# aikiriao/AAD

Measured on AMD Instinct MI355X. Metric: Msamples/s encode+decode, 48 kHz stereo 4-bit, higher is better.
Workload: dtype int32

## Files before the change

aad_amd/capi.py:

```python
import ctypes as C
import os

import numpy as np


class AADApiResult:
    OK = 0
    INVALID_ARGUMENT = 1
    INVALID_FORMAT = 2
    INSUFFICIENT_BUFFER = 3
    INSUFFICIENT_DATA = 4
    PARAMETER_NOT_SET = 5
    NG = 6
    _names = {0: "OK", 1: "INVALID_ARGUMENT", 2: "INVALID_FORMAT", 3: "INSUFFICIENT_BUFFER",
              4: "INSUFFICIENT_DATA", 5: "PARAMETER_NOT_SET", 6: "NG"}

    @classmethod
    def name(cls, v):
        return cls._names.get(int(v), str(v))


class AADHeaderInfo(C.Structure):
    _fields_ = [("format_version", C.c_uint32), ("codec_version", C.c_uint32),
                ("num_channels", C.c_uint16), ("num_samples", C.c_uint32),
# ... 23 lines not shown

class AADHipPlanarOutput(C.Structure):
    _fields_ = [("sample_type", C.c_int32), ("reserved", C.c_uint32), ("stream_stride", C.c_uint64), ("channel_stride", C.c_uint64)]


class AADHipRowStats(C.Structure):
    _fields_ = [("sum_sq", C.c_uint64), ("sum_abs", C.c_uint64), ("max_abs", C.c_uint64), ("count", C.c_uint64)]


class AADHipLaneState(C.Structure):
    _fields_ = [("weight", C.c_int32 * 4), ("history", C.c_int32 * 4),
                ("stepsize_index", C.c_int32), ("quantize_error", C.c_int32)]


STREAM_DESC_DTYPE = np.dtype([("pcm_offset", "<u8"), ("data_offset", "<u8"), ("data_size", "<u8"),
                              ("num_samples", "<u4"), ("reserved", "<u4")])
ERROR_STATS_DTYPE = np.dtype([("rms_error", "<f8"), ("mean_abs_error", "<f8"), ("max_abs_error", "<f8")])
WINDOW_DTYPE = np.dtype([("stream", "<i8"), ("first_frame", "<i8")])
SAMPLE_INT16, SAMPLE_FLOAT32 = 0, 1
RECONSTRUCT_DECODED, RECONSTRUCT_RESIDUAL = 0, 1
OPTION_LANE_MAPPING, OPTION_TRIAL_LANES, OPTION_STAGING_THREADS, OPTION_TILE_KBYTES, OPTION_COMPARE_ORDER = 0, 1, 2, 3, 4
LANE_MAPPINGS = {"auto": 0, "dense": 1, "quad": 2, "quad-fused": 3, "dense-tiled": 4}
TRIAL_LANES = {"dual": 0, "single": 1}
LANE_STATE_DTYPE = np.dtype([("weight", "<i4", (4,)), ("history", "<i4", (4,)),
                             ("stepsize_index", "<i4"), ("quantize_error", "<i4")])

_PKG_DIR = os.path.dirname(os.path.abspath(__file__))
LIBRARY_PATH = os.environ.get("AAD_HIP_LIBRARY", os.path.join(_PKG_DIR, "libaad_hip.so"))

LEGACY_SYMBOLS = [
    "AADEncoder_CalculateBlockSize", "AADEncoder_EncodeHeader", "AADEncoder_CalculateWorkSize",
    "AADEncoder_Create", "AADEncoder_Destroy", "AADEncoder_SetEncodeParameter", "AADEncoder_EncodeWhole",
    "AADDecoder_DecodeHeader", "AADDecoder_CalculateWorkSize", "AADDecoder_Create", "AADDecoder_Destroy",
    "AADDecoder_SetHeader", "AADDecoder_DecodeBlock", "AADDecoder_DecodeWhole",
]
HIP_SYMBOLS = [
    "AADHip_GetDeviceCount", "AADHip_ContextCreate", "AADHip_ContextDestroy", "AADHip_ContextSynchronize",
    "AADHip_ContextLastError", "AADHip_ContextSignalNextRun", "AADHip_SignalNextRunSupported", "AADHip_ContextSetOption", "AADHip_CalculateEncodedSize", "AADHip_EncodePlanCreate",
    "AADHip_EncodePlanDestroy", "AADHip_EncodePlanRun", "AADHip_DecodePlanCreate", "AADHip_DecodePlanDestroy",
    "AADHip_DecodePlanRun", "AADHip_EncodeBatch", "AADHip_DecodeBatch",
    "AADHip_ReconstructPlanCreate", "AADHip_ReconstructPlanDestroy", "AADHip_ReconstructPlanRun",
    "AADHip_ReconstructBatch", "AADHip_SegmentedEncodePlanCreate", "AADHip_SegmentedEncodeBatch",
    "AADHip_SegmentedReconstructPlanCreate", "AADHip_SegmentedReconstructBatch",
    "AADHip_WindowDecodePlanCreate", "AADHip_WindowDecodePlanDestroy", "AADHip_WindowDecodePlanRun",
    "AADHip_WindowDecodePlanRunStats", "AADHip_MixedWindowDecodePlanCreate", "AADHip_ChannelMixWindowDecodePlanCreate",
    "AADHip_PlanarEncodePlanCreate", "AADHip_PlanarEncodePlanRun",
# ... 257 lines not shown
```

aad_amd/csrc/aad_decode_split.hip:

```cpp
#include <cstring>

#include "aad_decode_split.hip.h"
#include "aad_launch.h"

namespace aad {

template <int BITS, bool LDSRES>
static void launch_bits(const SplitDecodeArgs &sa, dim3 grid, dim3 block, hipStream_t stream)
{
  if (sa.d.channels == 1)
    AAD_LAUNCH((decode_split_kernel<BITS, 1, false, LDSRES>), grid, block, 0, stream, sa);
  else if (sa.d.mid_side)
    AAD_LAUNCH((decode_split_kernel<BITS, 2, true, LDSRES>), grid, block, 0, stream, sa);
  else
    AAD_LAUNCH((decode_split_kernel<BITS, 2, false, LDSRES>), grid, block, 0, stream, sa);
}

void launch_decode_split(const DecodeArgs &args, const DecodeLaunch &p, int32_t *residual, hipStream_t stream)
{
  SplitDecodeArgs sa;
  sa.d = args;
  sa.residual = residual;
  sa.residual_stride = p.residual_stride;
  sa.reserved = 0;
  const dim3 grid(p.grid), block(p.workgroup);
  const bool lds = p.kernel == DecodeKernel::SplitLds;
  switch (args.bits) {
    case 4: lds ? launch_bits<4, true>(sa, grid, block, stream) : launch_bits<4, false>(sa, grid, block, stream); break;
    case 3: lds ? launch_bits<3, true>(sa, grid, block, stream) : launch_bits<3, false>(sa, grid, block, stream); break;
    default: lds ? launch_bits<2, true>(sa, grid, block, stream) : launch_bits<2, false>(sa, grid, block, stream); break;
  }
}

}

#if AAD_PHASE_TIMING
extern "C" uint32_t AADHipDebug_ReadSplitPhaseTimes(uint64_t *out, uint32_t capacity)
{
  uint32_t n = 0, zero = 0;
  uint64_t host[512];
  (void)hipDeviceSynchronize();
  (void)hipMemcpyFromSymbol(&n, HIP_SYMBOL(aad::g_phase_count), sizeof(n));
  (void)hipMemcpyFromSymbol(host, HIP_SYMBOL(aad::g_phase_times), sizeof(host));
  (void)hipMemcpyToSymbol(HIP_SYMBOL(aad::g_phase_count), &zero, sizeof(zero));
  if (n > capacity) n = capacity;
  memcpy(out, host, sizeof(uint64_t) * n);
  return n;
}
#endif
```

aad_amd/csrc/aad_decode_split.hip.h:

```cpp
#ifndef AAD_DECODE_SPLIT_HIP_H
#define AAD_DECODE_SPLIT_HIP_H

#include "aad_decode.hip.h"

namespace aad {

struct SplitDecodeArgs {
  DecodeArgs d;
  int32_t *residual;
  uint32_t residual_stride;
  uint32_t reserved;
};

struct BlockRef {
  const uint8_t *src;
  uint64_t pcm_first;
  uint32_t n;
  uint32_t avail;
};

__device__ __forceinline__ BlockRef locate_block(const DecodeArgs &a, uint64_t g, uint32_t ch)
{
  uint32_t s;
  StreamDesc sd;
  uint64_t b;
  if (a.uni.enabled) {
    s = (uint32_t)g / a.uni.blocks_per_stream;
    b = (uint32_t)g - s * a.uni.blocks_per_stream;
    sd = uniform_stream(a.uni, s);
  } else {
    s = find_stream(a.block_prefix, a.num_streams, g);
    sd = a.streams[s];
    b = g - a.block_prefix[s];
  }
// ... 284 lines not shown
    }
  }
  int32_t p = full ? C.p : predict(L);
  const uint32_t rem = coded - full * kChunk;
  if (rem) {
    ChunkResiduals last;
    last.load(res + full * kChunk);
    static_for<0, kChunk - 1>([&](auto jc) {
      constexpr int j = decltype(jc)::value;
      if ((uint32_t)j < rem) {
        const int32_t qd = last.get(j);
        const int32_t yy = clip16(qd + p);
        lms_and_shift<kShiftSelect>(L, qd, yy);
        p = predict(L);
        const int32_t yo = finish(yy);
        if (writer) dst[(uint64_t)(kTaps + full * kChunk + j) * ch] = (int16_t)yo;
      }
    });
  }
  AAD_PHASE_MARK(blockIdx.x == 0 && threadIdx.x == 0);
}


template <int BITS, int CHF, bool MS, bool LDSRES>
__global__ void __launch_bounds__(1024) decode_split_kernel(SplitDecodeArgs a)
{
  __shared__ uint32_t s_step[AAD_STEP_TABLE_LEN];
  __shared__ int32_t s_delta[8];
  __shared__ __attribute__((aligned(16))) int32_t s_res[LDSRES ? 16 * kLdsResidualRow : 4];
  __shared__ __attribute__((aligned(16))) uint32_t s_stage[2 * 16 * 8];
  AAD_PHASE_MARK(blockIdx.x == 0 && threadIdx.x == 0);
  for (uint32_t i = threadIdx.x; i < AAD_STEP_TABLE_LEN; i += blockDim.x) s_step[i] = c_step_table[i];
  if (threadIdx.x < 8) {
    const int16_t *dt = BITS == 4 ? c_delta4 : (BITS == 3 ? c_delta3 : c_delta2);
    s_delta[threadIdx.x] = dt[threadIdx.x & Pack<BITS>::kMagMax];
  }
  AAD_PHASE_MARK(blockIdx.x == 0 && threadIdx.x == 0);
  __syncthreads();
  AAD_PHASE_MARK(blockIdx.x == 0 && threadIdx.x == 0);
  {
    const uint32_t w = threadIdx.x >> 6;
    const uint64_t rec = (uint64_t)blockIdx.x * 16u + w;
    if (rec < a.d.total_blocks * CHF)
      residuals_for_recurrence<BITS>(a, rec, threadIdx.x & 63u, s_step, s_delta,
                                     LDSRES ? s_res + w * kLdsResidualRow : a.residual + rec * a.residual_stride);
  }
  AAD_PHASE_MARK(blockIdx.x == 0 && threadIdx.x == 0);
  __syncthreads();
  AAD_PHASE_MARK(blockIdx.x == 0 && threadIdx.x == 0);
  if (threadIdx.x >= 64) return;
  const uint64_t thread = (uint64_t)blockIdx.x * 64u + threadIdx.x;
  const uint64_t rec = thread >> 2;
  const bool active = rec < a.d.total_blocks * CHF;
  predict_for_quad<CHF, MS>(a, thread,
                            LDSRES ? s_res + (threadIdx.x >> 2) * kLdsResidualRow
                                   : a.residual + (active ? rec : 0) * a.residual_stride,
                            s_stage);
}

}

#endif
```

aad_amd/csrc/aad_device.hip.h:

```cpp
#ifndef AAD_DEVICE_HIP_H
#define AAD_DEVICE_HIP_H

#include <hip/hip_runtime.h>
#include <stdint.h>
#include <type_traits>

#include "aad_lds_layout.h"
#include "aad_tables_data.h"

#ifndef AAD_PHASE_TIMING
#define AAD_PHASE_TIMING 0
#endif

namespace aad {

#if AAD_PHASE_TIMING
static __device__ uint64_t g_phase_times[512];
static __device__ uint32_t g_phase_count;
__device__ __forceinline__ void phase_mark(bool who)
{
  if (who) {
    const uint32_t i = g_phase_count;
    if (i < 512) {
      g_phase_times[i] = __builtin_amdgcn_s_memtime();
// ... 73 lines not shown
  int32_t h0, h1, h2, h3;
  int32_t idxb;
};

template <int I, int N, class F>
__device__ __forceinline__ void static_for(F &&f)
{
  if constexpr (I < N) {
    f(std::integral_constant<int, I>{});
    static_for<I + 1, N>(f);
  }
}

template <int BITS>
struct Pack {
  static constexpr int kUnitSamples = BITS == 3 ? 8 : (BITS == 4 ? 2 : 4);
  static constexpr int kUnitBytes = BITS == 3 ? 3 : 1;
  static constexpr int kChunkBytes = kChunk * BITS / 8;
  static constexpr int kWords = BITS == 2 ? 1 : 2;
  static constexpr int kCodesPerWord = kChunk / kWords;
  static constexpr uint32_t kSign = 1u << (BITS - 1), kMagMax = kSign - 1u;
  static constexpr int pos(int j) { return BITS * (kCodesPerWord - 1 - j); }
};

template <int BITS, bool QUAD, int WIDE_STEP_SHIFT = 0, bool WIDE4 = false>
__device__ __forceinline__ void stage_tables(char *lds)
{
  constexpr int kShift = BITS - 1;
  auto put = [&](int i, uint32_t step_i, uint32_t recip_i) {
    const float hr = __uint_as_float(recip_i);
    const float hs = hr * (float)(1 << kShift);
    reinterpret_cast<uint32_t *>(lds + kLdsStepOff)[i] = step_i;
    reinterpret_cast<float *>(lds + kLdsHrOff)[i] = hr;
    reinterpret_cast<float *>(lds + kLdsHsOff)[i] = hs;
    if (QUAD) {
      u32x4 e;
      e.x = step_i << WIDE_STEP_SHIFT;
      e.y = __float_as_uint(hr);
      e.z = __float_as_uint(hs);
      e.w = 0;
      if (WIDE4) {
#pragma unroll
        for (int r = 0; r < kWideCopies; r++)
          *reinterpret_cast<u32x4 *>(lds + kLdsWideOff + i * (16 * kWideCopies) + (((r + i) & (kWideCopies - 1)) << 4)) = e;
      } else {
        *reinterpret_cast<u32x4 *>(lds + kLdsWideOff + (i << 4)) = e;
// ... 303 lines not shown
```

aad_amd/csrc/aad_encode.hip.h:

```cpp
#ifndef AAD_ENCODE_HIP_H
#define AAD_ENCODE_HIP_H

#include "aad_device.hip.h"
#include "aad_pcm_convert.h"
#include "aad_segments.h"

namespace aad {

constexpr bool kEncTM = true;

template <int BITS>
__device__ __forceinline__ int32_t index_delta_arith(uint32_t mag)
{
  if (BITS == 4) {
    const uint32_t corr = __builtin_amdgcn_perm(0u, 0x00161514u, mag) & 0xFFu;
    return (int32_t)(2u << mag) - (int32_t)corr;
  } else if (BITS == 3) {
    return mag < 2 ? (int32_t)mag - 16 : (int32_t)(2u << (2u * mag));
  } else {
    return mag ? 40 : -14;
  }
}

template <int BITS>
// ... 194 lines not shown
}


struct EncodeArgs {
  union {
    const StreamDesc *streams;
    const ChainDesc *chains;
  };
  const int16_t *pcm;
  uint8_t *data;
  const LaneStateRecord *state;
  LaneStateRecord *state_out;
  uint32_t num_streams;
  uint32_t channels;
  uint32_t block_size;
  uint32_t samples_per_block;
  uint32_t mid_side;
  uint32_t trials;
  uint32_t bits;
  uint32_t lead_frames;
  uint32_t ring_ok;
  uint8_t *trial_scratch;
  uint32_t trial_slot_bytes;
  UniformLayout uni;
  alignas(4) uint8_t header_template[32];
};

enum PcmLayout { kInInterleaved = 0, kInPlanarI16 = 1, kInPlanarF32 = 2 };
template <int IN> using PcmElem = std::conditional_t<IN == kInPlanarF32, float, int16_t>;

struct PlanarEncodeArgs : EncodeArgs {
  uint64_t channel_stride;
};
template <int IN> using EncodeArgsFor = std::conditional_t<IN == kInInterleaved, EncodeArgs, PlanarEncodeArgs>;

enum RecOutput { kRecNone = 0, kRecI16 = 1, kRecF32 = 2, kRecI16Stats = 3, kRecF32Stats = 4, kRecStatsOnly = 5 };
constexpr bool rec_has_stats(int rec) { return rec >= kRecI16Stats; }
constexpr int rec_rows(int rec) { return rec == kRecI16Stats ? kRecI16 : (rec == kRecF32Stats ? kRecF32 : (rec == kRecStatsOnly ? kRecNone : rec)); }

struct RecEncodeArgs : PlanarEncodeArgs {
  void *out;
  const uint64_t *out_base;
  uint64_t out_channel_stride;
};
struct StatsEncodeArgs : RecEncodeArgs {
  AADHipRowStats *stats;
// ... 1380 lines not shown
      if (qb != q) reinterpret_cast<U32x3 *>(img + 12u * qb)->v = ob;
      if (qc != q) reinterpret_cast<U32x3 *>(img + 12u * qc)->v = oc;
    }
    for (uint32_t o = pieces * 12u + id; o < used; o += kGroup) {
      const uint32_t owner = CHF == 2 ? ((o - kBlockHeaderBytesPerCh * ch) / UB) & 1u : 0u;
      img[o] = (owner ? s1 : s0)[o];
    }
  }
  F = from_quad<kEncTM>(best_end);
  last_qd = best_qd;
}

template <int BITS, int CHF, bool MS, bool QUAD, bool TRIALS, bool DUAL = false, bool RING = false, bool SEG = false, int IN = kInInterleaved,
          int REC = kRecNone>
__global__ void __launch_bounds__(256) encode_streams_kernel(KernelArgsFor<IN, REC> a)
{
  static_assert(REC == kRecNone || (!DUAL && !RING), "the decoded rows: single-layout trial search, plain stores");
  static_assert(!QUAD || CHF != 0, "the quad mapping exists for the mono / stereo fast paths");
  static_assert(!DUAL || (QUAD && TRIALS), "the dual mapping is the trial search on the quad mapping");
  static_assert(!RING || kRingable<BITS, CHF, QUAD>, "the byte ring: dense mono / stereo encoders");
  static_assert(!(SEG && RING), "segmented plans never take the byte ring");
  __shared__ __attribute__((aligned(16))) char lds[kLdsBytesEncoderStatic<BITS, CHF, QUAD, RING>];
  extern __shared__ __attribute__((aligned(16))) char ring_lds[];
  AAD_PHASE_MARK(blockIdx.x == 0 && threadIdx.x == 0);
  stage_tables<BITS, true, kWideStepShift, true>(lds);
  AAD_PHASE_MARK(blockIdx.x == 0 && threadIdx.x == 0);

  const uint32_t ch = CHF ? CHF : a.channels;
  const uint64_t thread = (uint64_t)blockIdx.x * blockDim.x + threadIdx.x;
  constexpr uint32_t kQuadsPerStream = DUAL ? 2u * (CHF ? CHF : 1) : 1u;
  const uint64_t slot = QUAD ? (thread >> 6) * 16u + quad_slot<kEncTM>() : thread;
  const uint32_t role = DUAL ? (uint32_t)(slot % kQuadsPerStream) / (CHF ? CHF : 1) : 0u;
  const uint64_t lane = DUAL ? slot / kQuadsPerStream * (CHF ? CHF : 1) + slot % (CHF ? CHF : 1)
                             : slot;
  const uint32_t tap = QUAD ? quad_tap<kEncTM>() : 0u;
  const bool writer = tap == 0 && role == 0;
  if (lane >= (uint64_t)a.num_streams * ch) return;
  const uint32_t s = (uint32_t)(lane / ch), c = (uint32_t)(lane % ch);
  StreamDesc sd;
  uint64_t block0 = 0;
  uint64_t warm_end = 0;
  bool head = true;
  uint32_t head_samples = 0;
  if constexpr (SEG) {
    const ChainDesc cd = a.chains[s];
    sd.pcm_offset = cd.pcm_offset;
    sd.data_offset = cd.data_offset;
    sd.data_size = 0;
    sd.num_samples = cd.num_frames;
    sd.reserved = 0;
    block0 = cd.first_block;
    warm_end = (uint64_t)cd.warmup_blocks * a.samples_per_block;
// ... 142 lines not shown
```

aad_amd/csrc/aad_hip_engine.hip:

```cpp
#include <hip/hip_runtime.h>

#include <cstdio>
#include <cstdlib>
#include <cstring>
#include <algorithm>
#include <condition_variable>
#include <functional>
#include <mutex>
#include <new>
#include <thread>
#include <vector>

#include "../../include/aad_hip.h"
#include "aad_compare.hip.h"
#include "aad_launch.h"
#include "aad_decode.hip.h"
#include "aad_decode_window.hip.h"
#include "aad_decode_window_mixed.hip.h"
#include "aad_decode_window_channel_mix.hip.h"
#include "aad_encode.hip.h"
#include "aad_encode_launch.hip.h"
#include "aad_format.h"
#include "aad_hip_internal.h"
#include "aad_tiles.h"
// ... 348 lines not shown
  if (*buf) {
    if (!hip_ok(ctx, hipStreamSynchronize(ctx->stream), "hipStreamSynchronize")) return false;
    (void)hipFree(*buf);
    *buf = nullptr;
    *capacity = 0;
  }
  if (!hip_ok(ctx, hipMalloc((void **)buf, bytes), what)) return false;
  *capacity = bytes;
  return true;
}

AADApiResult run_encode(AADHipContext *ctx, const aad::EncodeRun &run)
{
  if (run.args.num_streams == 0) return AAD_APIRESULT_OK;
  if (run.args.bits < 2 || run.args.bits > 4) return AAD_APIRESULT_INVALID_FORMAT;
  aad::EncodeRun r = run;
  aad::EncodeArgs &a = r.args;
  if ((reinterpret_cast<uintptr_t>(a.data) & 63u) != 0) a.ring_ok = 0;
  const aad::EncodeBatch batch{a.bits, a.channels, a.num_streams, a.trials, a.block_size, a.ring_ok != 0};
  const aad::EncodeLaunch p = r.rec != aad::kRecNone ? aad::plan_reconstruct_encode(ctx->device_info, ctx->knobs, batch)
                                                     : aad::plan_encode(ctx->device_info, ctx->knobs, batch);
  a.trial_scratch = nullptr;
  a.trial_slot_bytes = p.trial_slot_bytes;
  if (p.trial_scratch_bytes != 0) {
    if (!scratch_reserve(ctx, &ctx->d_trial, &ctx->trial_capacity, p.trial_scratch_bytes, "hipMalloc trial scratch")) return AAD_APIRESULT_NG;
    a.trial_scratch = ctx->d_trial;
  }
  auto by_layout = [&](auto rec) {
    constexpr int REC = decltype(rec)::value;
    switch (r.in) {
      case aad::kInPlanarF32: aad::launch_encode_run<aad::kInPlanarF32, REC>(r, p, ctx->stream); break;
      case aad::kInPlanarI16: aad::launch_encode_run<aad::kInPlanarI16, REC>(r, p, ctx->stream); break;
      case aad::kInInterleaved: aad::launch_encode_run<aad::kInInterleaved, REC>(r, p, ctx->stream); break;
    }
  };
  switch (r.rec) {
    case aad::kRecStatsOnly: by_layout(std::integral_constant<int, aad::kRecStatsOnly>{}); break;
    case aad::kRecF32Stats: by_layout(std::integral_constant<int, aad::kRecF32Stats>{}); break;
    case aad::kRecI16Stats: by_layout(std::integral_constant<int, aad::kRecI16Stats>{}); break;
    case aad::kRecF32: by_layout(std::integral_constant<int, aad::kRecF32>{}); break;
    case aad::kRecI16: by_layout(std::integral_constant<int, aad::kRecI16>{}); break;
    case aad::kRecNone: by_layout(std::integral_constant<int, aad::kRecNone>{}); break;
  }
  return hip_ok(ctx, hipGetLastError(), "encode launch") ? AAD_APIRESULT_OK : AAD_APIRESULT_NG;
}

// ... 324 lines not shown
{
  if (ctx == nullptr) return AAD_APIRESULT_INVALID_ARGUMENT;
  if (ctx->signal_refused && (hip_start_event != nullptr || hip_stop_event != nullptr)) {
    snprintf(ctx->last_error, sizeof(ctx->last_error),
             "AADHip_ContextSignalNextRun: refused, ROC_SYSTEM_SCOPE_SIGNAL=0 (device-scope completion signals: a wait on the "
             "run's event from another stream would never return); record an event behind the run instead");
    return AAD_APIRESULT_NG;
  }
  ctx->signal_next = aad::LaunchSignal{static_cast<hipEvent_t>(hip_start_event), static_cast<hipEvent_t>(hip_stop_event)};
  return AAD_APIRESULT_OK;
}

AADApiResult AADHip_ContextSetOption(struct AADHipContext *ctx, int32_t option, int32_t value)
{
  if (ctx == nullptr) return AAD_APIRESULT_INVALID_ARGUMENT;
  switch (option) {
    case AAD_HIP_OPTION_LANE_MAPPING:
      if (value < AAD_HIP_LANE_MAPPING_AUTO || value > AAD_HIP_LANE_MAPPING_DENSE_TILED) return AAD_APIRESULT_INVALID_ARGUMENT;
      ctx->knobs.lane_mapping = value;
      return AAD_APIRESULT_OK;
    case AAD_HIP_OPTION_TRIAL_LANES:
      if (value != AAD_HIP_TRIAL_LANES_DUAL && value != AAD_HIP_TRIAL_LANES_SINGLE) return AAD_APIRESULT_INVALID_ARGUMENT;
      ctx->knobs.trial_lanes = value;
      return AAD_APIRESULT_OK;
    case AAD_HIP_OPTION_COMPARE_ORDER:
      if (value != 0 && value != 1) return AAD_APIRESULT_INVALID_ARGUMENT;
      ctx->compare_sequential = value;
      return AAD_APIRESULT_OK;
    case AAD_HIP_OPTION_STAGING_THREADS:
      if (value < 0 || value > 8) return AAD_APIRESULT_INVALID_ARGUMENT;
      ctx->staging_threads = value;
      return AAD_APIRESULT_OK;
    case AAD_HIP_OPTION_TILE_KBYTES:
      if (value < 0) return AAD_APIRESULT_INVALID_ARGUMENT;
      ctx->tile_bytes = (int64_t)value << 10;
      return AAD_APIRESULT_OK;
    default:
      return AAD_APIRESULT_INVALID_ARGUMENT;
  }
}

uint64_t AADHip_CalculateEncodedSize(const struct AADEncodeParameter *parameter, uint32_t num_samples)
{
  AADHeaderInfo h;
  if (num_samples == 0) return 0;
  if (AADFormat_ParameterToHeader(parameter, num_samples, AAD_HIP_MAX_NUM_CHANNELS, &h) != AAD_APIRESULT_OK) return 0;
// ... 1541 lines not shown
```

aad_amd/csrc/aad_launch_policy.h:

```cpp
#ifndef AAD_LAUNCH_POLICY_H
#define AAD_LAUNCH_POLICY_H

#include <stdint.h>

#include "../../include/aad_hip.h"
#include "aad_lds_layout.h"

namespace aad {

struct Device {
  uint32_t cus, lds_per_cu;
};

struct Knobs {
  int32_t lane_mapping = AAD_HIP_LANE_MAPPING_AUTO;
  int32_t trial_lanes = AAD_HIP_TRIAL_LANES_DUAL;
  int32_t encode_ring = 1;
  int32_t encode_lds_pad = -1;
  int32_t decode_lds_pad = -1;
  uint64_t decode_nt_min = 0;
};

struct EncodeBatch {
  uint32_t bits, channels, streams, trials, block_size;
  bool ring_ok;
};

struct DecodeBatch {
  uint64_t blocks;
  uint32_t streams, channels, bits, samples_per_block, block_size, code_phase_uniform;
  bool pcm_aligned16, pcm_base_aligned16, stream_stores;
};

enum class EncodeKernel { Dense, DenseRing, Quad, QuadDual };
struct EncodeLaunch {
  EncodeKernel kernel;
  bool trials;
  uint32_t workgroup, grid, lds, trial_slot_bytes;
  uint64_t trial_scratch_bytes;
};

enum class DecodeKernel { SplitLds, SplitScratch, QuadFused, Tiled, Dense };
struct DecodeLaunch {
  DecodeKernel kernel;
  bool stream_stores;
  uint32_t workgroup, grid, lds, residual_stride;
  uint64_t residual_bytes;
};

constexpr uint32_t kSimdsPerCu = 4, kWaveLanes = 64;

inline uint64_t one_wave_per_simd(const Device &d) { return (uint64_t)d.cus * kSimdsPerCu * kWaveLanes; }

inline uint32_t pick_workgroup(const Device &d, uint64_t threads) { return threads <= one_wave_per_simd(d) ? 64u : 256u; }

inline uint32_t grid_for(uint64_t threads, uint32_t workgroup) { return (uint32_t)((threads + workgroup - 1) / workgroup); }

constexpr uint64_t kDualMaxRecurrences = 5120;
constexpr uint64_t kMaxTrialScratchBytes = 1ull << 30;

template <int BITS>
constexpr uint32_t dense_encoder_lds_of(uint32_t ch) { return ch == 1 ? kLdsBytesEncoder<BITS, 1, false> : ch == 2 ? kLdsBytesEncoder<BITS, 2, false> : kLdsBytesEncoder<BITS, 0, false>; }
inline uint32_t dense_encoder_lds(uint32_t bits, uint32_t ch) { return bits == 4 ? dense_encoder_lds_of<4>(ch) : bits == 3 ? dense_encoder_lds_of<3>(ch) : dense_encoder_lds_of<2>(ch); }

inline uint32_t dense_encode_workgroup(const Device &d, uint64_t lanes, uint32_t lds_one_wave)
{
  const uint32_t wg = pick_workgroup(d, lanes);
  if (wg != 64u) return wg;
  const uint64_t waves = (lanes + 63u) / 64u;
  const uint64_t resident = (uint64_t)d.cus * (d.lds_per_cu / ((lds_one_wave + 1023u) & ~1023u));
  return waves > resident ? 256u : 64u;
}

inline bool encode_ring_wanted(const Knobs &k, uint32_t bits, uint32_t channels, uint32_t workgroup)
{
  if (k.encode_ring != 1) return k.encode_ring == 2;
  return workgroup == 256u && (channels == 1 || bits == 4);
}

// ... 6 lines not shown
}

inline EncodeLaunch plan_encode(const Device &d, const Knobs &k, const EncodeBatch &b)
{
  EncodeLaunch p = {};
  const uint64_t lanes = (uint64_t)b.streams * b.channels;
  const int32_t m = b.channels > 2 ? AAD_HIP_LANE_MAPPING_DENSE : k.lane_mapping;
  const bool quad = m == AAD_HIP_LANE_MAPPING_QUAD || m == AAD_HIP_LANE_MAPPING_QUAD_FUSED || (m == AAD_HIP_LANE_MAPPING_AUTO && lanes <= one_wave_per_simd(d) / 4);
  p.trials = b.trials != 0;
  if (quad && p.trials && k.trial_lanes != AAD_HIP_TRIAL_LANES_SINGLE && lanes <= kDualMaxRecurrences) {
    const uint32_t slot = (b.block_size + 16u + 63u) & ~63u;
    const uint64_t want = (uint64_t)b.streams * 3u * slot;
    if (want <= kMaxTrialScratchBytes) {
      p.trial_slot_bytes = slot;
      p.trial_scratch_bytes = want;
    }
  }
  if (quad) {
    const bool dual = p.trial_scratch_bytes != 0;
    const uint64_t threads = lanes * (dual ? 8 : 4);
    p.kernel = dual ? EncodeKernel::QuadDual : EncodeKernel::Quad;
    p.workgroup = dual && threads <= 128ull * d.cus ? 128u : pick_workgroup(d, threads);
    p.grid = grid_for(threads, p.workgroup);
    return p;
  }
  p.kernel = EncodeKernel::Dense;
  uint32_t static_lds = dense_encoder_lds(b.bits, b.channels);
  p.workgroup = dense_encode_workgroup(d, lanes, static_lds);
  p.grid = grid_for(lanes, p.workgroup);
  if (p.trials) return p;
  if (b.ring_ok && b.channels <= 2 && encode_ring_wanted(k, b.bits, b.channels, p.workgroup)) {
    p.kernel = EncodeKernel::DenseRing;
    p.lds = (p.workgroup / 64u) * (uint32_t)(b.channels == 1 ? kLdsRingBytesPerWave<1> : kLdsRingBytesPerWave<2>);
    static_lds = (uint32_t)kLdsCodeStageOff + p.lds;
  }
  if (p.workgroup == 256u) p.lds += dense_encode_lds_pad(d, k, b.bits, lanes, static_lds);
  return p;
}

inline EncodeLaunch plan_reconstruct_encode(const Device &d, const Knobs &k, const EncodeBatch &b)
{
  Knobs r = k;
  r.trial_lanes = AAD_HIP_TRIAL_LANES_SINGLE;
  r.encode_ring = 0;
  return plan_encode(d, r, b);
}
// ... 49 lines not shown
  if (a.bits == 3 && !(a.code_phase_uniform == 1 || (a.code_phase_uniform == 2 && a.blocks <= a.streams))) return false;
  return true;
}

inline uint32_t dense_decode_lds_pad(const Device &d, const Knobs &k, uint64_t lanes, uint32_t channels, uint32_t bits)
{
  if (k.decode_lds_pad >= 0) return (uint32_t)k.decode_lds_pad;
  const bool gains = channels == 1 || (channels == 2 && bits != 4);
  return gains && lanes >= one_wave_per_simd(d) ? d.lds_per_cu / 2 - (uint32_t)kLdsBytesDenseDec : 0u;
}

inline DecodeLaunch plan_decode(const Device &d, const Knobs &k, const DecodeBatch &b)
{
  DecodeLaunch p = {};
  const uint64_t lanes = b.blocks * b.channels;
  const int32_t m = b.channels > 2 ? AAD_HIP_LANE_MAPPING_DENSE : k.lane_mapping;
  bool quad = m == AAD_HIP_LANE_MAPPING_QUAD_FUSED;
  if (m == AAD_HIP_LANE_MAPPING_QUAD || (m == AAD_HIP_LANE_MAPPING_AUTO && lanes <= kDecodeSplitMax)) {
    const uint64_t coded = b.samples_per_block > 4 ? (uint64_t)b.samples_per_block - 4 : 0;
    const uint64_t row = (coded + 15u) / 16u * 16u + 16u;
    if (row <= kMaxResidualBytes / sizeof(int32_t) && lanes * row * sizeof(int32_t) <= kMaxResidualBytes) {
      p.workgroup = 1024;
      p.grid = grid_for(lanes, 16);
      if (decode_split_fits_lds(d, b)) {
        p.kernel = DecodeKernel::SplitLds;
      } else {
        p.kernel = DecodeKernel::SplitScratch;
        p.residual_stride = (uint32_t)row;
        p.residual_bytes = lanes * row * sizeof(int32_t);
      }
      return p;
    }
    quad = m == AAD_HIP_LANE_MAPPING_QUAD;
  } else if (!quad && m != AAD_HIP_LANE_MAPPING_DENSE &&
             (m == AAD_HIP_LANE_MAPPING_DENSE_TILED || lanes >= tiled_decode_min(d, b.bits, b.channels)) && decode_tiled_applicable(b)) {
    p.kernel = DecodeKernel::Tiled;
    p.workgroup = kWaveLanes * kTiledWaves;
    p.grid = grid_for(lanes, p.workgroup);
    return p;
  }
  const uint64_t threads = quad ? lanes * 4 : lanes;
  p.kernel = quad ? DecodeKernel::QuadFused : DecodeKernel::Dense;
  p.workgroup = pick_workgroup(d, threads);
  p.grid = grid_for(threads, p.workgroup);
  if (quad) return p;
  p.stream_stores = b.stream_stores && b.channels == 2 && b.bits != 3 && lanes >= k.decode_nt_min;
  if (p.workgroup == 256u) p.lds = dense_decode_lds_pad(d, k, lanes, b.channels, b.bits);
  return p;
// ... 201 lines not shown
```

aad_amd/engine.py:

```python
import ctypes as C

import numpy as np

from .capi import (AADApiResult, AADHeaderInfo, AADHipPlanarLayout, AADHipPlanarOutput, AADHipSegmentation, ApiError, ERROR_STATS_DTYPE, LANE_MAPPINGS, LANE_STATE_DTYPE,
                   OPTION_COMPARE_ORDER, OPTION_LANE_MAPPING, OPTION_STAGING_THREADS, OPTION_TILE_KBYTES, OPTION_TRIAL_LANES, RECONSTRUCT_DECODED, RECONSTRUCT_RESIDUAL,
                   SAMPLE_FLOAT32, SAMPLE_INT16, STREAM_DESC_DTYPE, TRIAL_LANES, WINDOW_DTYPE, load_library, make_parameter)


def _check(where, rc):
    if rc != AADApiResult.OK:
        raise ApiError(where, rc)


def _round_up(v, a):
    return (v + a - 1) // a * a


class Engine:

    def __init__(self, device=0, stream="torch", lib=None):
        import torch
        if not torch.cuda.is_available():
            raise RuntimeError("aad_amd.Engine needs a HIP device (torch.cuda.is_available() is False)")
        self.torch = torch
        self.lib = lib or load_library()
        self.device = int(device)
        torch.cuda.set_device(self.device)
        if stream == "torch":
            cur = torch.cuda.current_stream(self.device)
# ... 33 lines not shown
                                                    stop.handle if stop is not None else None))

    def last_error(self):
        return (self.lib.AADHip_ContextLastError(self._ctx) or b"").decode()

    def set_mapping(self, mapping="auto", trial_lanes=None):
        _check("AADHip_ContextSetOption",
               self.lib.AADHip_ContextSetOption(self._ctx, OPTION_LANE_MAPPING, LANE_MAPPINGS[mapping or "auto"]))
        if trial_lanes is not None:
            _check("AADHip_ContextSetOption",
                   self.lib.AADHip_ContextSetOption(self._ctx, OPTION_TRIAL_LANES, TRIAL_LANES[trial_lanes]))

    def set_staging_threads(self, threads=0):
        _check("AADHip_ContextSetOption",
               self.lib.AADHip_ContextSetOption(self._ctx, OPTION_STAGING_THREADS, int(threads)))

    def set_tile_kbytes(self, kbytes=0):
        _check("AADHip_ContextSetOption",
               self.lib.AADHip_ContextSetOption(self._ctx, OPTION_TILE_KBYTES, int(kbytes)))

    def set_compare_order(self, sequential=False):
        _check("AADHip_ContextSetOption",
               self.lib.AADHip_ContextSetOption(self._ctx, OPTION_COMPARE_ORDER, 1 if sequential else 0))

    def synchronize(self):
        _check("AADHip_ContextSynchronize", self.lib.AADHip_ContextSynchronize(self._ctx))

    def encoded_size(self, param, num_samples):
        return int(self.lib.AADHip_CalculateEncodedSize(C.byref(param), num_samples))

    def encode_plan(self, param, descs, segment_blocks=None, warmup_blocks=0):
        descs = np.ascontiguousarray(descs, dtype=STREAM_DESC_DTYPE)
        plan = C.c_void_p()
        if segment_blocks is None:
            _check("AADHip_EncodePlanCreate",
                   self.lib.AADHip_EncodePlanCreate(self._ctx, C.byref(param), len(descs), descs.ctypes.data, C.byref(plan)))
        else:
            seg = AADHipSegmentation(int(segment_blocks), int(warmup_blocks))
            _check("AADHip_SegmentedEncodePlanCreate",
                   self.lib.AADHip_SegmentedEncodePlanCreate(self._ctx, C.byref(param), C.byref(seg), len(descs),
                                                             descs.ctypes.data, C.byref(plan)))
        p = EncodePlan(self, plan, param, descs)
        p.segmented = segment_blocks is not None
        return p

    def planar_encode_plan(self, param, descs, channel_stride, dtype, segment_blocks=None, warmup_blocks=0):
# ... 734 lines not shown
        ms = C.c_float()
        rc = self.runtime().hipEventElapsedTime(C.byref(ms), self.handle, stop.handle)
        if rc != 0:
            raise RuntimeError("hipEventElapsedTime failed (%d)" % rc)
        return float(ms.value)

    def synchronize(self):
        rc = self.runtime().hipEventSynchronize(self.handle)
        if rc != 0:
            raise RuntimeError("hipEventSynchronize failed (%d)" % rc)

    def close(self):
        if self.handle:
            self.runtime().hipEventDestroy(self.handle)
            self.handle = C.c_void_p()

    def __del__(self):
        try:
            self.close()
        except Exception:
            pass


class EncodeDecodePipeline:

    def __init__(self, enc_engine, dec_engine, param, streams, samples, ring=8):
        assert ring >= 2 and ring % 2 == 0
        assert enc_engine.stream.cuda_stream != dec_engine.stream.cuda_stream, "the two contexts need streams of their own"
        torch = enc_engine.torch
        self.torch, self.ring, self.k = torch, ring, 0
        self.enc_engine, self.dec_engine = enc_engine, dec_engine
        self.enc = enc_engine.uniform_encode_plan(param, streams, samples)
        self.images = [torch.zeros((streams, self.enc.stride), dtype=torch.uint8, device="cuda:%d" % enc_engine.device)
                       for _ in range(ring)]
        zero = torch.zeros((streams, samples, param.num_channels), dtype=torch.int16, device=self.images[0].device)
        self.enc.run(zero, self.images[0])
        torch.cuda.synchronize()
        self.header = parse_header(bytes(self.images[0][0, :31].cpu().numpy()))
        self.dec = dec_engine.uniform_decode_plan(self.header, streams, self.enc.stride, self.enc.image_size)
        self.encoded = [HipEvent() for _ in range(ring)]
        self.decoded = [torch.cuda.Event() for _ in range(ring)]

    def step(self, pcm, out, timing=None):
        k, ring = self.k, self.ring
        self.k += 1
        b = k % ring
        s_enc, s_dec = self.enc_engine.stream, self.dec_engine.stream
        if k >= ring and k % (ring // 2) == 0:
            s_enc.wait_event(self.decoded[(k - ring // 2 - 1) % ring])
        encoded = self.encoded[b] if timing is None else timing[1]
        self.enc_engine.signal_next(encoded, start=None if timing is None else timing[0])
        self.enc.run(pcm, self.images[b], None, ordered=False)
        encoded.wait_on(s_dec)
        if timing is not None:
            self.dec_engine.signal_next(timing[3], start=timing[2])
        self.dec.run(self.images[b], out, ordered=False)
        self.decoded[b].record(s_dec)
        return self.images[b]

    def close(self):
        self.torch.cuda.synchronize()
        self.enc.close()
        self.dec.close()
        for e in self.encoded:
            e.close()


def parse_header(data):
    if len(data) < 31 or data[:4] != b"AAD\x00":
        raise ApiError("parse_header", AADApiResult.INVALID_FORMAT)
    be = lambda o, n: int.from_bytes(data[o:o + n], "big")
    return AADHeaderInfo(format_version=be(4, 4), codec_version=be(8, 4), num_channels=be(12, 2),
                         num_samples=be(14, 4), sampling_rate=be(18, 4), bits_per_sample=be(22, 2),
                         block_size=be(24, 2), num_samples_per_block=be(26, 4), ch_process_method=data[30])


__all__ = ["Engine", "EncodePlan", "PlanarEncodePlan", "PlanarReconstructPlan", "DecodePlan", "WindowDecodePlan", "EncodeDecodePipeline", "parse_header", "make_parameter", "LANE_STATE_DTYPE", "rmse", "snr_db", "level_dbfs", "select_least_bits"]
```

include/aad_hip.h:

```cpp
#ifndef AAD_HIP_H_INCLUDED
#define AAD_HIP_H_INCLUDED

#include <stdint.h>
#include "aad.h"
#include "aad_encoder.h"

#define AAD_HIP_MAX_NUM_CHANNELS 8

struct AADHipContext;
struct AADHipEncodePlan;
struct AADHipDecodePlan;

struct AADHipStreamDesc {
  uint64_t pcm_offset;
  uint64_t data_offset;
  uint64_t data_size;
  uint32_t num_samples;
  uint32_t reserved;
};

struct AADHipLaneState {
  int32_t weight[4];
  int32_t history[4];
  int32_t stepsize_index;
  int32_t quantize_error;
};

#ifdef __cplusplus
extern "C" {
#endif

int32_t AADHip_GetDeviceCount(void);

AADApiResult AADHip_ContextCreate(int32_t device_index, void *hip_stream, struct AADHipContext **context);
void AADHip_ContextDestroy(struct AADHipContext *context);
AADApiResult AADHip_ContextSynchronize(struct AADHipContext *context);
const char *AADHip_ContextLastError(const struct AADHipContext *context);

AADApiResult AADHip_ContextSignalNextRun(struct AADHipContext *context, void *hip_start_event, void *hip_stop_event);
int32_t AADHip_SignalNextRunSupported(void);

enum AADHipOption {
  AAD_HIP_OPTION_LANE_MAPPING = 0,
  AAD_HIP_OPTION_TRIAL_LANES = 1,
  AAD_HIP_OPTION_STAGING_THREADS = 2,
  AAD_HIP_OPTION_TILE_KBYTES = 3,
  AAD_HIP_OPTION_COMPARE_ORDER = 4
};
enum AADHipLaneMapping {
  AAD_HIP_LANE_MAPPING_AUTO = 0,
  AAD_HIP_LANE_MAPPING_DENSE = 1,
  AAD_HIP_LANE_MAPPING_QUAD = 2,
  AAD_HIP_LANE_MAPPING_QUAD_FUSED = 3,
  AAD_HIP_LANE_MAPPING_DENSE_TILED = 4
};
enum AADHipTrialLanes {
  AAD_HIP_TRIAL_LANES_DUAL = 0,
  AAD_HIP_TRIAL_LANES_SINGLE = 1
};
AADApiResult AADHip_ContextSetOption(struct AADHipContext *context, int32_t option, int32_t value);

uint64_t AADHip_CalculateEncodedSize(const struct AADEncodeParameter *parameter, uint32_t num_samples);


AADApiResult AADHip_EncodePlanCreate(
    struct AADHipContext *context, const struct AADEncodeParameter *parameter,
    uint32_t num_streams, const struct AADHipStreamDesc *streams,
    struct AADHipEncodePlan **plan);
void AADHip_EncodePlanDestroy(struct AADHipEncodePlan *plan);

// ... 191 lines not shown
```

Baseline: 102,500.

## Pin encode and decode work to disjoint SIMDs when pipelined

Adds a SIMD-role option. Each wave reads its hardware SIMD id, and work is routed so that encode uses one SIMD pair of each CU and decode uses the other. The encode quad kernel launches 256-thread groups and keeps only the wave that lands on the wanted SIMD. The split decode kernel spreads its residual phase over waves on the matching SIMD parity and elects a worker wave on the chosen SIMD, sizing its LDS dynamically. The pipeline turns this on by default through a per-device allocator, aiming to stop the concurrent encode and decode streams from contending for the same SIMDs. In exchange it launches extra idle waves and does less parallel residual work per block.

```diff
diff --git a/aad_amd/capi.py b/aad_amd/capi.py
--- a/aad_amd/capi.py
+++ b/aad_amd/capi.py
@@ -69,6 +69,8 @@
 OPTION_LANE_MAPPING, OPTION_TRIAL_LANES, OPTION_STAGING_THREADS, OPTION_TILE_KBYTES, OPTION_COMPARE_ORDER = 0, 1, 2, 3, 4
 LANE_MAPPINGS = {"auto": 0, "dense": 1, "quad": 2, "quad-fused": 3, "dense-tiled": 4}
 TRIAL_LANES = {"dual": 0, "single": 1}
+OPTION_SIMD_ROLE = 5
+SIMD_ROLE_OFF = -1
 LANE_STATE_DTYPE = np.dtype([("weight", "<i4", (4,)), ("history", "<i4", (4,)),
                              ("stepsize_index", "<i4"), ("quantize_error", "<i4")])
 
diff --git a/aad_amd/csrc/aad_decode_split.hip b/aad_amd/csrc/aad_decode_split.hip
--- a/aad_amd/csrc/aad_decode_split.hip
+++ b/aad_amd/csrc/aad_decode_split.hip
@@ -5,9 +5,28 @@
 
 namespace aad {
 
+constexpr uint32_t kRoleLdsMax = 16u * (kLdsResidualMax + 4u) * (uint32_t)sizeof(int32_t);
+
+template <int BITS, int CHF, bool MS, bool LDSRES>
+static void launch_role(const SplitDecodeArgs &sa, dim3 grid, dim3 block, uint32_t lds, hipStream_t stream)
+{
+  if constexpr (LDSRES) {
+    static const hipError_t raised = hipFuncSetAttribute(reinterpret_cast<const void *>(&decode_split_kernel<BITS, CHF, MS, true, true>),
+                                                         hipFuncAttributeMaxDynamicSharedMemorySize, (int)kRoleLdsMax);
+    (void)raised;
+  }
+  AAD_LAUNCH((decode_split_kernel<BITS, CHF, MS, LDSRES, true>), grid, block, lds, stream, sa);
+}
+
 template <int BITS, bool LDSRES>
-static void launch_bits(const SplitDecodeArgs &sa, dim3 grid, dim3 block, hipStream_t stream)
+static void launch_bits(const SplitDecodeArgs &sa, dim3 grid, dim3 block, uint32_t role_lds, bool role, hipStream_t stream)
 {
+  if (role) {
+    if (sa.d.channels == 1) launch_role<BITS, 1, false, LDSRES>(sa, grid, block, role_lds, stream);
+    else if (sa.d.mid_side) launch_role<BITS, 2, true, LDSRES>(sa, grid, block, role_lds, stream);
+    else launch_role<BITS, 2, false, LDSRES>(sa, grid, block, role_lds, stream);
+    return;
+  }
   if (sa.d.channels == 1)
     AAD_LAUNCH((decode_split_kernel<BITS, 1, false, LDSRES>), grid, block, 0, stream, sa);
   else if (sa.d.mid_side)
@@ -22,13 +41,16 @@
   sa.d = args;
   sa.residual = residual;
   sa.residual_stride = p.residual_stride;
+  const bool role = p.simd_role != 0;
+  sa.simd = role ? (uint8_t)(p.simd_role - 1u) : 0;
   sa.reserved = 0;
+  sa.lds_row = (uint16_t)p.lds_row;
   const dim3 grid(p.grid), block(p.workgroup);
   const bool lds = p.kernel == DecodeKernel::SplitLds;
   switch (args.bits) {
-    case 4: lds ? launch_bits<4, true>(sa, grid, block, stream) : launch_bits<4, false>(sa, grid, block, stream); break;
-    case 3: lds ? launch_bits<3, true>(sa, grid, block, stream) : launch_bits<3, false>(sa, grid, block, stream); break;
-    default: lds ? launch_bits<2, true>(sa, grid, block, stream) : launch_bits<2, false>(sa, grid, block, stream); break;
+    case 4: lds ? launch_bits<4, true>(sa, grid, block, p.lds, role, stream) : launch_bits<4, false>(sa, grid, block, 0, role, stream); break;
+    case 3: lds ? launch_bits<3, true>(sa, grid, block, p.lds, role, stream) : launch_bits<3, false>(sa, grid, block, 0, role, stream); break;
+    default: lds ? launch_bits<2, true>(sa, grid, block, p.lds, role, stream) : launch_bits<2, false>(sa, grid, block, 0, role, stream); break;
   }
 }
 
diff --git a/aad_amd/csrc/aad_decode_split.hip.h b/aad_amd/csrc/aad_decode_split.hip.h
--- a/aad_amd/csrc/aad_decode_split.hip.h
+++ b/aad_amd/csrc/aad_decode_split.hip.h
@@ -9,7 +9,8 @@
   DecodeArgs d;
   int32_t *residual;
   uint32_t residual_stride;
-  uint32_t reserved;
+  uint8_t simd, reserved;
+  uint16_t lds_row;
 };
 
 struct BlockRef {
@@ -340,13 +341,18 @@
 }
 
 
-template <int BITS, int CHF, bool MS, bool LDSRES>
+template <int BITS, int CHF, bool MS, bool LDSRES, bool ROLE = false>
 __global__ void __launch_bounds__(1024) decode_split_kernel(SplitDecodeArgs a)
 {
   __shared__ uint32_t s_step[AAD_STEP_TABLE_LEN];
   __shared__ int32_t s_delta[8];
-  __shared__ __attribute__((aligned(16))) int32_t s_res[LDSRES ? 16 * kLdsResidualRow : 4];
+  __shared__ __attribute__((aligned(16))) int32_t s_res_static[LDSRES && !ROLE ? 16 * kLdsResidualRow : 4];
+  extern __shared__ __attribute__((aligned(16))) int32_t s_res_dynamic[];
   __shared__ __attribute__((aligned(16))) uint32_t s_stage[2 * 16 * 8];
+  __shared__ uint32_t s_wave_simd[ROLE ? 16 : 1];
+  int32_t *const s_res = ROLE && LDSRES ? s_res_dynamic : s_res_static;
+  const uint32_t res_row = ROLE ? a.lds_row : kLdsResidualRow;
+  if constexpr (ROLE) publish_wave_simd(s_wave_simd);
   AAD_PHASE_MARK(blockIdx.x == 0 && threadIdx.x == 0);
   for (uint32_t i = threadIdx.x; i < AAD_STEP_TABLE_LEN; i += blockDim.x) s_step[i] = c_step_table[i];
   if (threadIdx.x < 8) {
@@ -356,22 +362,43 @@
   AAD_PHASE_MARK(blockIdx.x == 0 && threadIdx.x == 0);
   __syncthreads();
   AAD_PHASE_MARK(blockIdx.x == 0 && threadIdx.x == 0);
-  {
-    const uint32_t w = threadIdx.x >> 6;
+  uint32_t first = threadIdx.x >> 6, stride = 16;
+  if constexpr (ROLE) {
+    uint32_t rank = 0, count = 0;
+    bool mine = false;
+    for (uint32_t w = 0; w < 16u; w++) {
+      const bool on_pair = ((s_wave_simd[w] ^ a.simd) & 1u) == 0;
+      if (w == (threadIdx.x >> 6)) {
+        mine = on_pair;
+        rank = count;
+      }
+      count += on_pair;
+    }
+    if (count) {
+      first = mine ? rank : 16u;
+      stride = count;
+    }
+  }
+  for (uint32_t w = first; w < 16u; w += stride) {
     const uint64_t rec = (uint64_t)blockIdx.x * 16u + w;
     if (rec < a.d.total_blocks * CHF)
       residuals_for_recurrence<BITS>(a, rec, threadIdx.x & 63u, s_step, s_delta,
-                                     LDSRES ? s_res + w * kLdsResidualRow : a.residual + rec * a.residual_stride);
+                                     LDSRES ? s_res + w * res_row : a.residual + rec * a.residual_stride);
   }
   AAD_PHASE_MARK(blockIdx.x == 0 && threadIdx.x == 0);
   __syncthreads();
   AAD_PHASE_MARK(blockIdx.x == 0 && threadIdx.x == 0);
-  if (threadIdx.x >= 64) return;
-  const uint64_t thread = (uint64_t)blockIdx.x * 64u + threadIdx.x;
+  if constexpr (ROLE) {
+    if ((threadIdx.x >> 6) != elected_worker_wave(a.simd, s_wave_simd)) return;
+  } else {
+    if (threadIdx.x >= 64) return;
+  }
+  const uint32_t lane = threadIdx.x & 63u;
+  const uint64_t thread = (uint64_t)blockIdx.x * 64u + lane;
   const uint64_t rec = thread >> 2;
   const bool active = rec < a.d.total_blocks * CHF;
   predict_for_quad<CHF, MS>(a, thread,
-                            LDSRES ? s_res + (threadIdx.x >> 2) * kLdsResidualRow
+                            LDSRES ? s_res + (lane >> 2) * res_row
                                    : a.residual + (active ? rec : 0) * a.residual_stride,
                             s_stage);
 }
diff --git a/aad_amd/csrc/aad_device.hip.h b/aad_amd/csrc/aad_device.hip.h
--- a/aad_amd/csrc/aad_device.hip.h
+++ b/aad_amd/csrc/aad_device.hip.h
@@ -119,6 +119,26 @@
   static constexpr uint32_t kSign = 1u << (BITS - 1), kMagMax = kSign - 1u;
   static constexpr int pos(int j) { return BITS * (kCodesPerWord - 1 - j); }
 };
+
+__device__ __forceinline__ uint32_t wave_simd_id() { return __builtin_amdgcn_s_getreg(4 | (4 << 6) | (1 << 11));  }
+__device__ __forceinline__ void publish_wave_simd(uint32_t *slot)
+{
+  if ((threadIdx.x & 63u) == 0) slot[threadIdx.x >> 6] = wave_simd_id();
+}
+__device__ __forceinline__ uint32_t elected_worker_wave(uint32_t wanted_simd, const uint32_t *slot)
+{
+  const uint32_t waves = blockDim.x >> 6;
+  uint32_t worker = 0;
+  for (uint32_t w = waves; w-- > 0;)
+    if (slot[w] == wanted_simd) worker = w;
+  return worker;
+}
+__device__ __forceinline__ uint32_t elect_worker_wave(uint32_t wanted_simd, uint32_t *slot)
+{
+  publish_wave_simd(slot);
+  __syncthreads();
+  return elected_worker_wave(wanted_simd, slot);
+}
 
 template <int BITS, bool QUAD, int WIDE_STEP_SHIFT = 0, bool WIDE4 = false>
 __device__ __forceinline__ void stage_tables(char *lds)
diff --git a/aad_amd/csrc/aad_encode.hip.h b/aad_amd/csrc/aad_encode.hip.h
--- a/aad_amd/csrc/aad_encode.hip.h
+++ b/aad_amd/csrc/aad_encode.hip.h
@@ -240,6 +240,7 @@
   uint32_t ring_ok;
   uint8_t *trial_scratch;
   uint32_t trial_slot_bytes;
+  uint32_t simd_role;
   UniformLayout uni;
   alignas(4) uint8_t header_template[32];
 };
@@ -1666,12 +1667,23 @@
   static_assert(!(SEG && RING), "segmented plans never take the byte ring");
   __shared__ __attribute__((aligned(16))) char lds[kLdsBytesEncoderStatic<BITS, CHF, QUAD, RING>];
   extern __shared__ __attribute__((aligned(16))) char ring_lds[];
+  constexpr bool kRoles = QUAD && !DUAL;
+  __shared__ uint32_t s_wave_simd[kRoles ? 4 : 1];
   AAD_PHASE_MARK(blockIdx.x == 0 && threadIdx.x == 0);
+  if constexpr (kRoles) {
+    if (a.simd_role) publish_wave_simd(s_wave_simd);
+  }
   stage_tables<BITS, true, kWideStepShift, true>(lds);
   AAD_PHASE_MARK(blockIdx.x == 0 && threadIdx.x == 0);
 
   const uint32_t ch = CHF ? CHF : a.channels;
-  const uint64_t thread = (uint64_t)blockIdx.x * blockDim.x + threadIdx.x;
+  uint64_t thread = (uint64_t)blockIdx.x * blockDim.x + threadIdx.x;
+  if constexpr (kRoles) {
+    if (a.simd_role) {
+      if ((threadIdx.x >> 6) != elected_worker_wave(a.simd_role - 1u, s_wave_simd)) return;
+      thread = (uint64_t)blockIdx.x * 64u + (threadIdx.x & 63u);
+    }
+  }
   constexpr uint32_t kQuadsPerStream = DUAL ? 2u * (CHF ? CHF : 1) : 1u;
   const uint64_t slot = QUAD ? (thread >> 6) * 16u + quad_slot<kEncTM>() : thread;
   const uint32_t role = DUAL ? (uint32_t)(slot % kQuadsPerStream) / (CHF ? CHF : 1) : 0u;
diff --git a/aad_amd/csrc/aad_hip_engine.hip b/aad_amd/csrc/aad_hip_engine.hip
--- a/aad_amd/csrc/aad_hip_engine.hip
+++ b/aad_amd/csrc/aad_hip_engine.hip
@@ -394,6 +394,7 @@
                                                      : aad::plan_encode(ctx->device_info, ctx->knobs, batch);
   a.trial_scratch = nullptr;
   a.trial_slot_bytes = p.trial_slot_bytes;
+  a.simd_role = p.simd_role;
   if (p.trial_scratch_bytes != 0) {
     if (!scratch_reserve(ctx, &ctx->d_trial, &ctx->trial_capacity, p.trial_scratch_bytes, "hipMalloc trial scratch")) return AAD_APIRESULT_NG;
     a.trial_scratch = ctx->d_trial;
@@ -764,6 +765,10 @@
     case AAD_HIP_OPTION_TRIAL_LANES:
       if (value != AAD_HIP_TRIAL_LANES_DUAL && value != AAD_HIP_TRIAL_LANES_SINGLE) return AAD_APIRESULT_INVALID_ARGUMENT;
       ctx->knobs.trial_lanes = value;
+      return AAD_APIRESULT_OK;
+    case AAD_HIP_OPTION_SIMD_ROLE:
+      if (value < AAD_HIP_SIMD_ROLE_OFF || value > AAD_HIP_SIMD_ROLE_3) return AAD_APIRESULT_INVALID_ARGUMENT;
+      ctx->knobs.simd_role = value;
       return AAD_APIRESULT_OK;
     case AAD_HIP_OPTION_COMPARE_ORDER:
       if (value != 0 && value != 1) return AAD_APIRESULT_INVALID_ARGUMENT;
diff --git a/aad_amd/csrc/aad_launch_policy.h b/aad_amd/csrc/aad_launch_policy.h
--- a/aad_amd/csrc/aad_launch_policy.h
+++ b/aad_amd/csrc/aad_launch_policy.h
@@ -19,6 +19,7 @@
   int32_t encode_lds_pad = -1;
   int32_t decode_lds_pad = -1;
   uint64_t decode_nt_min = 0;
+  int32_t simd_role = AAD_HIP_SIMD_ROLE_OFF;
 };
 
 struct EncodeBatch {
@@ -38,6 +39,7 @@
   bool trials;
   uint32_t workgroup, grid, lds, trial_slot_bytes;
   uint64_t trial_scratch_bytes;
+  uint32_t simd_role;
 };
 
 enum class DecodeKernel { SplitLds, SplitScratch, QuadFused, Tiled, Dense };
@@ -46,6 +48,7 @@
   bool stream_stores;
   uint32_t workgroup, grid, lds, residual_stride;
   uint64_t residual_bytes;
+  uint32_t simd_role, lds_row;
 };
 
 constexpr uint32_t kSimdsPerCu = 4, kWaveLanes = 64;
@@ -55,6 +58,14 @@
 inline uint32_t pick_workgroup(const Device &d, uint64_t threads) { return threads <= one_wave_per_simd(d) ? 64u : 256u; }
 
 inline uint32_t grid_for(uint64_t threads, uint32_t workgroup) { return (uint32_t)((threads + workgroup - 1) / workgroup); }
+
+inline uint32_t plan_simd_role(const Device &d, const Knobs &k, uint32_t workgroups)
+{
+  if (k.simd_role < 0 || k.simd_role >= (int32_t)kSimdsPerCu || workgroups > d.cus) return 0;
+  return 1u + (uint32_t)k.simd_role;
+}
+
+inline uint32_t split_lds_row(uint32_t coded) { return (coded + (uint32_t)kChunk - 1u) / (uint32_t)kChunk * (uint32_t)kChunk + 4u; }
 
 constexpr uint64_t kDualMaxRecurrences = 5120;
 constexpr uint64_t kMaxTrialScratchBytes = 1ull << 30;
@@ -107,6 +118,10 @@
     p.kernel = dual ? EncodeKernel::QuadDual : EncodeKernel::Quad;
     p.workgroup = dual && threads <= 128ull * d.cus ? 128u : pick_workgroup(d, threads);
     p.grid = grid_for(threads, p.workgroup);
+    if (!dual && p.workgroup == 64u) {
+      p.simd_role = plan_simd_role(d, k, p.grid);
+      if (p.simd_role) p.workgroup = 256u;
+    }
     return p;
   }
   p.kernel = EncodeKernel::Dense;
@@ -202,8 +217,13 @@
     if (row <= kMaxResidualBytes / sizeof(int32_t) && lanes * row * sizeof(int32_t) <= kMaxResidualBytes) {
       p.workgroup = 1024;
       p.grid = grid_for(lanes, 16);
+      p.simd_role = plan_simd_role(d, k, p.grid);
       if (decode_split_fits_lds(d, b)) {
         p.kernel = DecodeKernel::SplitLds;
+        if (p.simd_role) {
+          p.lds_row = split_lds_row((uint32_t)coded);
+          p.lds = 16u * p.lds_row * (uint32_t)sizeof(int32_t);
+        }
       } else {
         p.kernel = DecodeKernel::SplitScratch;
         p.residual_stride = (uint32_t)row;
diff --git a/aad_amd/engine.py b/aad_amd/engine.py
--- a/aad_amd/engine.py
+++ b/aad_amd/engine.py
@@ -3,8 +3,8 @@
 import numpy as np
 
 from .capi import (AADApiResult, AADHeaderInfo, AADHipPlanarLayout, AADHipPlanarOutput, AADHipSegmentation, ApiError, ERROR_STATS_DTYPE, LANE_MAPPINGS, LANE_STATE_DTYPE,
-                   OPTION_COMPARE_ORDER, OPTION_LANE_MAPPING, OPTION_STAGING_THREADS, OPTION_TILE_KBYTES, OPTION_TRIAL_LANES, RECONSTRUCT_DECODED, RECONSTRUCT_RESIDUAL,
-                   SAMPLE_FLOAT32, SAMPLE_INT16, STREAM_DESC_DTYPE, TRIAL_LANES, WINDOW_DTYPE, load_library, make_parameter)
+                   OPTION_COMPARE_ORDER, OPTION_LANE_MAPPING, OPTION_SIMD_ROLE, OPTION_STAGING_THREADS, OPTION_TILE_KBYTES, OPTION_TRIAL_LANES, RECONSTRUCT_DECODED, RECONSTRUCT_RESIDUAL,
+                   SAMPLE_FLOAT32, SAMPLE_INT16, SIMD_ROLE_OFF, STREAM_DESC_DTYPE, TRIAL_LANES, WINDOW_DTYPE, load_library, make_parameter)
 
 
 def _check(where, rc):
@@ -84,6 +84,10 @@
     def set_compare_order(self, sequential=False):
         _check("AADHip_ContextSetOption",
                self.lib.AADHip_ContextSetOption(self._ctx, OPTION_COMPARE_ORDER, 1 if sequential else 0))
+
+    def set_simd_role(self, simd=None):
+        _check("AADHip_ContextSetOption",
+               self.lib.AADHip_ContextSetOption(self._ctx, OPTION_SIMD_ROLE, SIMD_ROLE_OFF if simd is None else int(simd)))
 
     def synchronize(self):
         _check("AADHip_ContextSynchronize", self.lib.AADHip_ContextSynchronize(self._ctx))
@@ -864,14 +868,57 @@
             pass
 
 
+PIPELINE_SIMD_ROLES = True
+
+
+class SimdRoleAllocator:
+    SLOTS = ((0, 1), (2, 3))
+
+    def __init__(self):
+        self.taken = [False] * len(self.SLOTS)
+        self.holders = [None] * len(self.SLOTS)
+
+    def in_force(self):
+        return all(self.taken)
+
+    def acquire(self, apply=None):
+        for i, t in enumerate(self.taken):
+            if not t:
+                self.taken[i] = True
+                self.holders[i] = apply
+                self._apply_all()
+                return i
+        return None
+
+    def release(self, slot):
+        if slot is not None and self.taken[slot]:
+            apply = self.holders[slot]
+            self.taken[slot], self.holders[slot] = False, None
+            if apply is not None:
+                apply(None, None)
+            self._apply_all()
+
+    def roles(self, slot):
+        return self.SLOTS[slot] if slot is not None and self.taken[slot] and self.in_force() else (None, None)
+
+    def _apply_all(self):
+        for i, apply in enumerate(self.holders):
+            if self.taken[i] and apply is not None:
+                apply(*self.roles(i))
+
+
+_simd_roles = {}
+
+
 class EncodeDecodePipeline:
 
-    def __init__(self, enc_engine, dec_engine, param, streams, samples, ring=8):
+    def __init__(self, enc_engine, dec_engine, param, streams, samples, ring=8, simd_roles=PIPELINE_SIMD_ROLES):
         assert ring >= 2 and ring % 2 == 0
         assert enc_engine.stream.cuda_stream != dec_engine.stream.cuda_stream, "the two contexts need streams of their own"
         torch = enc_engine.torch
         self.torch, self.ring, self.k = torch, ring, 0
         self.enc_engine, self.dec_engine = enc_engine, dec_engine
+        self._take_simd_roles(_simd_roles.setdefault(enc_engine.device, SimdRoleAllocator()) if simd_roles else None)
         self.enc = enc_engine.uniform_encode_plan(param, streams, samples)
         self.images = [torch.zeros((streams, self.enc.stride), dtype=torch.uint8, device="cuda:%d" % enc_engine.device)
                        for _ in range(ring)]
@@ -906,6 +953,20 @@
         self.dec.close()
         for e in self.encoded:
             e.close()
+        self._release_simd_roles()
+
+    def _take_simd_roles(self, allocator):
+        self._roles = allocator
+        self._role_slot = allocator.acquire(self._set_simd_roles) if allocator is not None else None
+
+    def _set_simd_roles(self, enc_simd, dec_simd):
+        self.enc_engine.set_simd_role(enc_simd)
+        self.dec_engine.set_simd_role(dec_simd)
+
+    def _release_simd_roles(self):
+        if getattr(self, "_role_slot", None) is not None:
+            self._roles.release(self._role_slot)
+            self._role_slot = None
 
 
 def parse_header(data):
@@ -917,4 +978,4 @@
                          block_size=be(24, 2), num_samples_per_block=be(26, 4), ch_process_method=data[30])
 
 
-__all__ = ["Engine", "EncodePlan", "PlanarEncodePlan", "PlanarReconstructPlan", "DecodePlan", "WindowDecodePlan", "EncodeDecodePipeline", "parse_header", "make_parameter", "LANE_STATE_DTYPE", "rmse", "snr_db", "level_dbfs", "select_least_bits"]
+__all__ = ["Engine", "EncodePlan", "PlanarEncodePlan", "PlanarReconstructPlan", "DecodePlan", "WindowDecodePlan", "EncodeDecodePipeline", "SimdRoleAllocator", "parse_header", "make_parameter", "LANE_STATE_DTYPE", "rmse", "snr_db", "level_dbfs", "select_least_bits"]
diff --git a/include/aad_hip.h b/include/aad_hip.h
--- a/include/aad_hip.h
+++ b/include/aad_hip.h
@@ -45,7 +45,12 @@
   AAD_HIP_OPTION_TRIAL_LANES = 1,
   AAD_HIP_OPTION_STAGING_THREADS = 2,
   AAD_HIP_OPTION_TILE_KBYTES = 3,
-  AAD_HIP_OPTION_COMPARE_ORDER = 4
+  AAD_HIP_OPTION_COMPARE_ORDER = 4,
+  AAD_HIP_OPTION_SIMD_ROLE = 5
+};
+enum AADHipSimdRole {
+  AAD_HIP_SIMD_ROLE_OFF = -1,
+  AAD_HIP_SIMD_ROLE_0 = 0, AAD_HIP_SIMD_ROLE_1 = 1, AAD_HIP_SIMD_ROLE_2 = 2, AAD_HIP_SIMD_ROLE_3 = 3
 };
 enum AADHipLaneMapping {
   AAD_HIP_LANE_MAPPING_AUTO = 0,
```

New measurement: 119,400, median of 6. 1.17x the previous value.
